# loli/medpy

Measured on AMD Instinct MI355X. Metric: Mvoxels/s graph-cut (build+solve), 512^3 6-conn; fraction of HBM roofline, higher is better.
Workload: dtype f64

## Files before the change

include/medpy_hip.h:

```cpp
#ifndef MEDPY_HIP_H
#define MEDPY_HIP_H

#include <stdint.h>

#ifdef __cplusplus
extern "C" {
#endif

typedef struct mgc_graph* mgc_handle;

typedef enum mgc_status {
    MGC_OK = 0,
    MGC_ERR_INVALID = 1,
    MGC_ERR_NO_DEVICE = 2,
    MGC_ERR_HIP = 3,
    MGC_ERR_OOM = 4,
    MGC_ERR_STATE = 5,
    MGC_ERR_UNSUPPORTED = 6,
    MGC_ERR_NOT_CONVERGED = 7
} mgc_status;

typedef enum mgc_term {
    MGC_TERM_NONE = 0,
    MGC_TERM_DIFFERENCE_LINEAR = 1,
// ... 92 lines not shown
int mgc_get_nweights(mgc_handle h, int axis, double* out);
int mgc_get_tweights(mgc_handle h, double* out);
int mgc_get_nweights_offset(mgc_handle h, const int* offset, double* out);
int mgc_get_edge(mgc_handle h, int64_t i, int64_t j, double* out);

int mgc_maxflow(mgc_handle h, double* flow);

int mgc_labels(mgc_handle h, uint8_t* out);
int mgc_what_segment(mgc_handle h, int64_t i, int* segment);

int mgc_get_node_num(mgc_handle h, int64_t* n);
int mgc_set_param(mgc_handle h, const char* name, int64_t value);
int mgc_get_stats(mgc_handle h, mgc_stats* out);
int mgc_get_profile(mgc_handle h, uint64_t* out16);
enum {
    MGC_LAUNCH_DISCHARGE = 0,
    MGC_LAUNCH_DISCHARGE_W = 1,
    MGC_LAUNCH_RELABEL_TILE = 2,
    MGC_LAUNCH_RELABEL_V = 3,
    MGC_LAUNCH_RELABEL_W = 4,
    MGC_LAUNCH_DISCHARGE26 = 5,
    MGC_LAUNCH_DISCHARGE26_V = 6,
    MGC_LAUNCH_DISCHARGE26_W = 7,
    MGC_NLAUNCH = 8
};
int mgc_get_launch_counts(mgc_handle h, int64_t* out, int n);

enum {
    MGC_OP_ABSORB_ALL = 0,
    MGC_OP_FILL_INF = 1,
    MGC_OP_ZERO_COUNT = 2,
    MGC_OP_RELABEL_ALL = 3,
    MGC_OP_RELABEL_LIST = 4,
    MGC_OP_ACTIVATE = 5,
    MGC_OP_DISCHARGE = 6,
    MGC_OP_SUSPECT_PASS = 7,
    MGC_OP_RESET_SUSPECT = 8
};
int mgc_create_slab(int ndim, const int64_t* global_shape, int connectivity, int device, int rank, int nranks, mgc_handle* out);
int mgc_slab_info(mgc_handle h, int64_t* info8);
int mgc_solver_op(mgc_handle h, int op, int64_t a0, int64_t a1, int64_t a2, int64_t a3);
int mgc_read_counts(mgc_handle h, int32_t* out32);
int mgc_halo_bytes(mgc_handle h, int kind, int64_t* bytes);
int mgc_halo_pack(mgc_handle h, int side, int kind, void* buf, int buf_on_device);
int mgc_halo_unpack(mgc_handle h, int side, int kind, const void* buf, int buf_on_device, uint32_t epoch, int list);
int mgc_finish(mgc_handle h, double* flow_partial);

int mgc_comm_unique_id(uint8_t* id128);
int mgc_comm_init(mgc_handle h, const uint8_t* id128);
int mgc_halo_exchange(mgc_handle h, int kind, uint32_t epoch, int list);

typedef struct mgc_slab_stats {
    int64_t outer;
    int64_t relabel_passes;
    int64_t phases;
    int64_t exchanges;
    int64_t reductions;
    int64_t converged;
    int64_t discharge_tiles;
    int64_t relabel_tiles;
    int64_t deferred_drains;
    int64_t reserved[7];
} mgc_slab_stats;
int mgc_solve_slab(mgc_handle h, mgc_slab_stats* out);

// ... 57 lines not shown
```

medpy_amd/_lib.py:

```python
import ctypes as C
import os

import numpy as np

_HERE = os.path.dirname(os.path.abspath(__file__))
LIB_PATH = os.environ.get("MEDPY_HIP_LIB") or os.path.join(_HERE, "libmedpyhip.so")

OK, ERR_INVALID, ERR_NO_DEVICE, ERR_HIP, ERR_OOM, ERR_STATE, ERR_UNSUPPORTED, ERR_NOT_CONVERGED = range(8)

TERM_IDS = {
    "none": 0,
    "difference_linear": 1, "difference_exponential": 2, "difference_division": 3, "difference_power": 4,
    "maximum_linear": 5, "maximum_exponential": 6, "maximum_division": 7, "maximum_power": 8,
}

DTYPE_IDS = {
    np.dtype(np.uint8): 0, np.dtype(np.int8): 1, np.dtype(np.uint16): 2, np.dtype(np.int16): 3,
    np.dtype(np.uint32): 4, np.dtype(np.int32): 5, np.dtype(np.uint64): 6, np.dtype(np.int64): 7,
    np.dtype(np.float32): 8, np.dtype(np.float64): 9,
}


class Stats(C.Structure):
    _fields_ = [
        ("build_ms", C.c_double), ("solve_ms", C.c_double), ("discharge_ms", C.c_double), ("relabel_ms", C.c_double),
        ("discharge_launches", C.c_int64), ("relabel_launches", C.c_int64), ("discharge_tiles", C.c_int64),
        ("relabel_tiles", C.c_int64), ("global_relabels", C.c_int64), ("phases", C.c_int64), ("ntiles", C.c_int64),
        ("nvox", C.c_int64), ("device_bytes", C.c_int64), ("reserved", C.c_int64 * 3),
        ("discharge_wave_ms", C.c_double), ("discharge_wave_launches", C.c_int64), ("discharge_wave_tiles", C.c_int64),
        ("timing_stride", C.c_int64), ("update_ms", C.c_double), ("delta_ms", C.c_double),
    ]

    def as_dict(self):
        d = {k: getattr(self, k) for k, _ in self._fields_ if k != "reserved"}
        d["readbacks"] = self.reserved[0]
        d["radial_cycles"] = self.reserved[1]
        d["wall_tiles"] = self.reserved[2]
        return d


LAUNCH_KINDS = ("k_discharge", "k_discharge_w", "k_relabel_tile", "k_relabel_v", "k_relabel_w", "k26_discharge", "k26_discharge_v", "k26_discharge_w")


class Validation(C.Structure):
    _fields_ = [("voxels", C.c_int64), ("negative_values", C.c_int64), ("active_excess", C.c_int64),
                ("residual_arcs_across", C.c_int64), ("sink_links_across", C.c_int64), ("pair_violations", C.c_int64),
                ("node_violations", C.c_int64), ("pending_outbox", C.c_int64), ("reserved", C.c_int64 * 4),
                ("max_pair_error", C.c_double), ("max_node_error", C.c_double), ("flow_into_sink", C.c_double),
                ("cut_capacity", C.c_double), ("flow_constant", C.c_double), ("sink_capacity_used", C.c_double),
                ("reserved_d", C.c_double * 2)]

    def as_dict(self):
        return {k: getattr(self, k) for k, _ in self._fields_ if not k.startswith("reserved")}


VIOLATION_KEYS = ("negative_values", "active_excess", "residual_arcs_across", "sink_links_across", "pair_violations",
                  "node_violations", "pending_outbox")


def assert_valid(v, rel=1e-9):
    bad = {k: v[k] for k in VIOLATION_KEYS if v[k]}
    assert not bad, "max-flow invariants violated: %r" % (bad,)
    scale = max(abs(v["flow_into_sink"]), abs(v["cut_capacity"]), 1e-300)
    diff = abs(v["flow_into_sink"] - v["cut_capacity"])
# ... 52 lines not shown
    "mgc_labels_delta": (_INT, [_VP, _I64, _VP, C.POINTER(_I64)]),
    "mgc_add_edges": (_INT, [_VP, _I64, _VP, _VP, _VP, _VP]),
    "mgc_set_tweights_merged": (_INT, [_VP, _VP, _DBL]),
    "mgc_build": (_INT, [_VP]),
    "mgc_get_nweights": (_INT, [_VP, _INT, _VP]),
    "mgc_get_tweights": (_INT, [_VP, _VP]),
    "mgc_get_nweights_offset": (_INT, [_VP, C.POINTER(_INT), _VP]),
    "mgc_get_edge": (_INT, [_VP, _I64, _I64, C.POINTER(_DBL)]),
    "mgc_maxflow": (_INT, [_VP, C.POINTER(_DBL)]),
    "mgc_labels": (_INT, [_VP, _VP]),
    "mgc_what_segment": (_INT, [_VP, _I64, C.POINTER(_INT)]),
    "mgc_get_node_num": (_INT, [_VP, C.POINTER(_I64)]),
    "mgc_set_param": (_INT, [_VP, C.c_char_p, _I64]),
    "mgc_validate": (_INT, [_VP, _VP]),
    "mgc_get_image_range": (_INT, [_VP, _VP]),
    "mgc_set_image_range": (_INT, [_VP, _VP]),
    "mgc_get_stats": (_INT, [_VP, C.POINTER(Stats)]),
    "mgc_get_profile": (_INT, [_VP, _VP]),
    "mgc_get_launch_counts": (_INT, [_VP, _VP, _INT]),
    "mgc_create_slab": (_INT, [_INT, C.POINTER(_I64), _INT, _INT, _INT, _INT, C.POINTER(_VP)]),
    "mgc_slab_info": (_INT, [_VP, C.POINTER(_I64)]),
    "mgc_solver_op": (_INT, [_VP, _INT, _I64, _I64, _I64, _I64]),
    "mgc_read_counts": (_INT, [_VP, _VP]),
    "mgc_halo_bytes": (_INT, [_VP, _INT, C.POINTER(_I64)]),
    "mgc_halo_pack": (_INT, [_VP, _INT, _INT, _VP, _INT]),
    "mgc_halo_unpack": (_INT, [_VP, _INT, _INT, _VP, _INT, C.c_uint32, _INT]),
    "mgc_finish": (_INT, [_VP, C.POINTER(_DBL)]),
    "mgc_comm_unique_id": (_INT, [_VP]),
    "mgc_comm_init": (_INT, [_VP, _VP]),
    "mgc_halo_exchange": (_INT, [_VP, _INT, C.c_uint32, _INT]),
    "mgc_allreduce_counts": (_INT, [_VP, _VP]),
    "mgc_solve_slab": (_INT, [_VP, C.POINTER(SlabStats)]),
    "mgc_solve_slabs": (_INT, [C.POINTER(C.c_void_p), _INT, C.POINTER(Transport), C.POINTER(SlabStats)]),
    "msg_create": (_INT, [_I64, _INT, C.POINTER(_VP)]),
    "msg_destroy": (_INT, [_VP]),
    "msg_last_error": (C.c_char_p, [_VP]),
    "msg_set_param": (_INT, [_VP, C.c_char_p, _I64]),
    "msg_add_edges": (_INT, [_VP, _I64, _VP, _VP, _VP, _VP]),
    "msg_add_lattice_edges": (_INT, [_VP, _INT, _INT, C.POINTER(_I64), _VP, _INT, _DBL, C.POINTER(_DBL)]),
    "msg_add_label_edges": (_INT, [_VP, _INT, _INT, C.POINTER(_I64), _VP, _VP, _INT, _DBL]),
    "msg_region_sums": (_INT, [_INT, _I64, _VP, _VP, _INT, _INT, _I64, _VP, _VP]),
    "msg_set_tweights_merged": (_INT, [_VP, _VP, _DBL]),
    "msg_maxflow": (_INT, [_VP, C.POINTER(_DBL)]),
    "msg_labels": (_INT, [_VP, _VP]),
    "msg_what_segment": (_INT, [_VP, _I64, C.POINTER(_INT)]),
    "msg_get_edge": (_INT, [_VP, _I64, _I64, C.POINTER(_DBL)]),
# ... 76 lines not shown
```

medpy_amd/csrc/mgc_kernels.hip:

```cpp
#include <hip/hip_runtime.h>
#include <rccl/rccl.h>

#include <dlfcn.h>

#include <math.h>
#include <stdarg.h>
#include <stdio.h>
#include <stdlib.h>
#include <string.h>

#include <algorithm>
#include <map>
#include <string>
#include <mutex>
#include <thread>
#include <vector>

#include "../../include/medpy_hip.h"
#include "mgc_tile_ops.inl"
#include "mgc_tile_ops26.inl"
#include "mgc_wave_ops.inl"
#include "mgc_wave_ops26.inl"
#include "mgc_dt_ops.inl"
#include "mgc_brick_ops.inl"
// ... 798 lines not shown

__global__ __launch_bounds__(MGC_TV) void k_activate_list(MgcLattice L, int list, int cnt, uint32_t phase)
{
    __shared__ MgcTileShared S;
    GpuBlock x(S);
    MgcListView view;
    const int n = mgc_list_view(L, cnt, view);
    for (int i = blockIdx.x; i < n; i += gridDim.x) {
        x.new_tile();
        mgc_activate_tile(x, L, mgc_list_at(L, list, view, i), phase);
        __syncthreads();
    }
}

template <int AXIS, bool BWD, int SEED, int FINAL>
__global__ __launch_bounds__(256) void k_dt_scan(MgcLattice L, const void* in, void* out, int c_min, int32_t* hout, const uint16_t* carry_in, uint16_t* carry_out, int carry_plane)
{
    __shared__ MgcWaveShared S;
    GpuWave w(S);
    const int n = mgc_dt_lines<AXIS>(L);
    for (int line = (int)blockIdx.x * 4 + (int)(threadIdx.x >> 6); line < n; line += (int)gridDim.x * 4) {
        w.new_tile();
        mgc_dt_scan_line<AXIS, BWD, SEED, FINAL>(w, L, __builtin_amdgcn_readfirstlane(line), in, out, c_min, hout, carry_in, carry_out, carry_plane);
    }
}

__global__ __launch_bounds__(256) void k_shadow_sync(MgcLattice L)
{
    __shared__ MgcWaveShared S;
    GpuWave w(S);
    const int T = L.gy * L.gx;
    for (int i = (int)blockIdx.x * 4 + (int)(threadIdx.x >> 6); i < 2 * T; i += (int)gridDim.x * 4) {
        w.new_tile();
        mgc_shadow_sync_tile(w, L, i / T, __builtin_amdgcn_readfirstlane(i % T), L.height);
    }
}

__global__ __launch_bounds__(256) void k_dt_finish(MgcLattice L)
{
    __shared__ MgcWaveShared S;
    GpuWave w(S);
    if (blockIdx.x == 0 && threadIdx.x == 0) atomicAdd(&L.count[9], L.ntiles);
    for (int tile = (int)blockIdx.x * 4 + (int)(threadIdx.x >> 6); tile < L.ntiles; tile += (int)gridDim.x * 4) {
        w.new_tile();
        mgc_dt_finish_tile(w, L, __builtin_amdgcn_readfirstlane(tile));
    }
// ... 1647 lines not shown
            else hipLaunchKernelGGL(k_absorb_list, dim3(grid(h->L.ntiles)), dim3(MGC_TV), 0, h->stream, h->L, 6, fslot(0), fnext(0));
            filter_done(0, true);
            check(hipGetLastError());
        }
    }
    void relabel_all(uint32_t epoch, int next)
    {
        flush_zero();
        h->brick_mode = false;
        const int id = time_begin(1);
        if constexpr (FULL) hipLaunchKernelGGL(k26_relabel_all, dim3(grid(h->L.ntiles)), dim3(MGC_TV), 0, h->stream, h->L, epoch, next);
        else if (!(h->use_filters & 1)) { hipLaunchKernelGGL(k_relabel_all, dim3(grid(h->L.ntiles)), dim3(MGC_TV), 0, h->stream, h->L, epoch, next); h->launches[MGC_LAUNCH_RELABEL_TILE]++; }
        else {
            flush_zero();
            hipLaunchKernelGGL(k_filter, dim3(filter_grid()), dim3(256), 0, h->stream, h->L, 3, 6, fslot(0));
            if (h->wave_kernels & 8) { hipLaunchKernelGGL(k_relabel_v, dim3(grid(h->L.ntiles)), dim3(MGC_TV / MGC_RELABEL_V), 0, h->stream, h->L, 6, fslot(0), epoch, next, fnext(0), 1); filter_done(0, true); h->launches[MGC_LAUNCH_RELABEL_V]++; }
            else if (h->wave_kernels & 2) { hipLaunchKernelGGL(k_relabel_w, dim3(h->wave_grid_rel), dim3(MGCW_LANES), 0, h->stream, h->L, 6, fslot(0), epoch, next, -1, 1, h->tk_rel); h->tk_rel ^= 1; filter_done(0, false); h->launches[MGC_LAUNCH_RELABEL_W]++; }
            else { hipLaunchKernelGGL(k_relabel_first_list, dim3(grid(h->L.ntiles)), dim3(MGC_TV), 0, h->stream, h->L, 6, fslot(0), epoch, next); filter_done(0, false); h->launches[MGC_LAUNCH_RELABEL_TILE]++; }
        }
        check(hipGetLastError());
        time_end(id);
        relabel_launches++;
    }
    bool first_relabel_dt()
    {
        if (FULL || !h->use_dt || !h->all_residual || h->labels_valid || h->nranks > 1) return false;
        if (!h->d_dt16) {
            if (mgc_dmalloc((void**)&h->d_dt16, (size_t)h->L.ntiles * MGC_TV * sizeof(uint16_t)) != hipSuccess) { (void)hipGetLastError(); return false; }
            h->device_bytes += (int64_t)h->L.ntiles * MGC_TV * (int64_t)sizeof(uint16_t);
        }
        flush_zero();
        h->labels_valid = true;
        const int id = time_begin(2);
        const MgcLattice& L = h->L;
        void* const T = h->d_dt16;
        const dim3 blk(256);
        auto g = [&](int lines) { return dim3(grid((lines + 3) / 4)); };
        hipLaunchKernelGGL((k_dt_scan<0, false, 1, 0>), g(L.gz * L.gy), blk, 0, h->stream, L, (const void*)L.rmask, T, 0, (int32_t*)nullptr, (const uint16_t*)nullptr, (uint16_t*)nullptr, -1);
        hipLaunchKernelGGL((k_dt_scan<0, true, 0, 0>), g(L.gz * L.gy), blk, 0, h->stream, L, (const void*)T, T, 0, (int32_t*)nullptr, (const uint16_t*)nullptr, (uint16_t*)nullptr, -1);
        hipLaunchKernelGGL((k_dt_scan<1, false, 0, 0>), g(L.gz * L.gx), blk, 0, h->stream, L, (const void*)T, T, 0, (int32_t*)nullptr, (const uint16_t*)nullptr, (uint16_t*)nullptr, -1);
        hipLaunchKernelGGL((k_dt_scan<1, true, 0, 0>), g(L.gz * L.gx), blk, 0, h->stream, L, (const void*)T, T, 0, (int32_t*)nullptr, (const uint16_t*)nullptr, (uint16_t*)nullptr, -1);
        hipLaunchKernelGGL((k_dt_scan<2, false, 0, 0>), g(L.gy * L.gx), blk, 0, h->stream, L, (const void*)T, T, 0, (int32_t*)nullptr, (const uint16_t*)nullptr, (uint16_t*)nullptr, -1);
        hipLaunchKernelGGL((k_dt_scan<2, true, 0, 1>), g(L.gy * L.gx), blk, 0, h->stream, L, (const void*)T, (void*)L.height, 0, (int32_t*)nullptr, (const uint16_t*)nullptr, (uint16_t*)nullptr, -1);
        hipLaunchKernelGGL(k_dt_finish, g(L.ntiles), blk, 0, h->stream, L);
        check(hipGetLastError());
        time_end(id);
        relabel_launches += 7;
        return true;
    }
    void set_radial(bool on) { h->radial_on = on; if (on) h->radial_cycle_no++; }
    bool radial_begin(int c_min)
    {
        if (FULL) return false;
        const size_t nv = (size_t)h->L.ntiles * MGC_TV;
        if (!h->d_ds16) {
            if (mgc_dmalloc((void**)&h->d_ds16, nv * sizeof(uint16_t)) != hipSuccess) { (void)hipGetLastError(); return false; }
            h->device_bytes += (int64_t)(nv * sizeof(uint16_t));
        }
        if (!h->d_hexact) {
            if (mgc_dmalloc((void**)&h->d_hexact, nv * sizeof(int32_t)) != hipSuccess) { (void)hipGetLastError(); return false; }
            h->device_bytes += (int64_t)(nv * sizeof(int32_t));
        }
        flush_zero();
        const int id = time_begin(2);
        const MgcLattice& L = h->L;
        void* const T = h->d_ds16;
        const dim3 blk(256);
        auto g = [&](int lines) { return dim3(grid((lines + 3) / 4)); };
        check(hipMemsetAsync(L.count + mgc_cnt_radial_c(L), 0x3f, sizeof(int32_t), h->stream));
        hipLaunchKernelGGL(k_dt_cmin, g(L.ntiles), blk, 0, h->stream, L);
        hipLaunchKernelGGL((k_dt_scan<0, false, 2, 0>), g(L.gz * L.gy), blk, 0, h->stream, L, (const void*)L.excess, T, 0, (int32_t*)nullptr, (const uint16_t*)nullptr, (uint16_t*)nullptr, -1);
        hipLaunchKernelGGL((k_dt_scan<0, true, 0, 0>), g(L.gz * L.gy), blk, 0, h->stream, L, (const void*)T, T, 0, (int32_t*)nullptr, (const uint16_t*)nullptr, (uint16_t*)nullptr, -1);
        hipLaunchKernelGGL((k_dt_scan<1, false, 0, 0>), g(L.gz * L.gx), blk, 0, h->stream, L, (const void*)T, T, 0, (int32_t*)nullptr, (const uint16_t*)nullptr, (uint16_t*)nullptr, -1);
        hipLaunchKernelGGL((k_dt_scan<1, true, 0, 0>), g(L.gz * L.gx), blk, 0, h->stream, L, (const void*)T, T, 0, (int32_t*)nullptr, (const uint16_t*)nullptr, (uint16_t*)nullptr, -1);
        hipLaunchKernelGGL((k_dt_scan<2, false, 0, 0>), g(L.gy * L.gx), blk, 0, h->stream, L, (const void*)T, T, 0, (int32_t*)nullptr, (const uint16_t*)nullptr, (uint16_t*)nullptr, -1);
        hipLaunchKernelGGL((k_dt_scan<2, true, 0, 2>), g(L.gy * L.gx), blk, 0, h->stream, L, (const void*)T, T, c_min, h->d_hexact, (const uint16_t*)nullptr, (uint16_t*)nullptr, -1);
        std::swap(h->L.height, h->d_hexact);
        check(hipGetLastError());
        time_end(id);
        relabel_launches += 8;
        return true;
    }
    void radial_save_exact()
    {
        flush_zero();
        check(hipMemcpyAsync(h->d_hexact, h->L.height, (size_t)h->L.ntiles * MGC_TV * sizeof(int32_t), hipMemcpyDeviceToDevice, h->stream));
    }
    void radial_restore_exact()
    {
        flush_zero();
        std::swap(h->L.height, h->d_hexact);
    }
    void radial_lower(int c_min)
    {
        flush_zero();
        const int id = time_begin(2);
        hipLaunchKernelGGL(k_dt_lower, dim3(grid((h->L.ntiles + 3) / 4)), dim3(256), 0, h->stream, h->L, (const uint16_t*)h->d_ds16, c_min);
        check(hipGetLastError());
        time_end(id);
        relabel_launches++;
    }
    void source_open()
    {
// ... 104 lines not shown
    uint16_t* carry_buf(int dir) { return h->d_carry[dir]; }
    uint16_t* carry_recv_buf(int dir) { return h->d_carry_in[dir]; }
    bool ensure(void** p, size_t bytes)
    {
        if (*p) return true;
        if (mgc_dmalloc(p, bytes) != hipSuccess) { (void)hipGetLastError(); *p = nullptr; return false; }
        h->device_bytes += (int64_t)bytes;
        return true;
    }
    bool dt_applicable()
    {
        if (FULL || !h->use_dt || !h->all_residual || h->labels_valid) return false;
        bool ok = ensure((void**)&h->d_dt16, (size_t)h->L.ntiles * MGC_TV * sizeof(uint16_t));
        for (int k = 0; k < 2 && ok; ++k) ok = ensure((void**)&h->d_carry[k], (size_t)carry_bytes()) && ensure((void**)&h->d_carry_in[k], (size_t)carry_bytes());
        return ok;
    }
    dim3 dt_grid(int lines) const { return dim3(grid((lines + 3) / 4)); }
    int dt_span = -1;
    void dt_scans_xy(int seed)
    {
        flush_zero();
        h->labels_valid = true;
        dt_span = time_begin(2);
        const MgcLattice& L = h->L;
        void* const T = h->dt_cur = seed == 1 ? h->d_dt16 : h->d_ds16;
        const dim3 blk(256);
        if (seed == 1) hipLaunchKernelGGL((k_dt_scan<0, false, 1, 0>), dt_grid(L.gz * L.gy), blk, 0, h->stream, L, (const void*)L.rmask, T, 0, (int32_t*)nullptr, (const uint16_t*)nullptr, (uint16_t*)nullptr, -1);
        else hipLaunchKernelGGL((k_dt_scan<0, false, 2, 0>), dt_grid(L.gz * L.gy), blk, 0, h->stream, L, (const void*)L.excess, T, 0, (int32_t*)nullptr, (const uint16_t*)nullptr, (uint16_t*)nullptr, -1);
        hipLaunchKernelGGL((k_dt_scan<0, true, 0, 0>), dt_grid(L.gz * L.gy), blk, 0, h->stream, L, (const void*)T, T, 0, (int32_t*)nullptr, (const uint16_t*)nullptr, (uint16_t*)nullptr, -1);
        hipLaunchKernelGGL((k_dt_scan<1, false, 0, 0>), dt_grid(L.gz * L.gx), blk, 0, h->stream, L, (const void*)T, T, 0, (int32_t*)nullptr, (const uint16_t*)nullptr, (uint16_t*)nullptr, -1);
        hipLaunchKernelGGL((k_dt_scan<1, true, 0, 0>), dt_grid(L.gz * L.gx), blk, 0, h->stream, L, (const void*)T, T, 0, (int32_t*)nullptr, (const uint16_t*)nullptr, (uint16_t*)nullptr, -1);
        check(hipGetLastError());
        relabel_launches += 4;
    }
    void dt_scan_z(bool bwd, int final_kind, int c_min, const uint16_t* cin, bool want_out)
    {
        const MgcLattice& L = h->L;
        void* const T = h->dt_cur;
        const dim3 blk(256), g = dt_grid(L.gy * L.gx);
        uint16_t* const cout = want_out ? h->d_carry[bwd ? 1 : 0] : nullptr;
        const int plane = want_out ? carry_plane(bwd ? 1 : 0) : -1;
        if (!bwd) hipLaunchKernelGGL((k_dt_scan<2, false, 0, 0>), g, blk, 0, h->stream, L, (const void*)T, T, 0, (int32_t*)nullptr, cin, cout, plane);
        else if (final_kind == 1) hipLaunchKernelGGL((k_dt_scan<2, true, 0, 1>), g, blk, 0, h->stream, L, (const void*)T, (void*)L.height, 0, (int32_t*)nullptr, cin, cout, plane);
        else if (final_kind == 2) hipLaunchKernelGGL((k_dt_scan<2, true, 0, 2>), g, blk, 0, h->stream, L, (const void*)T, T, c_min, h->d_hexact, cin, cout, plane);
        else hipLaunchKernelGGL((k_dt_scan<2, true, 0, 0>), g, blk, 0, h->stream, L, (const void*)T, T, 0, (int32_t*)nullptr, cin, cout, plane);
        check(hipGetLastError());
        relabel_launches++;
        if (bwd) { time_end(dt_span); dt_span = -1; }
    }
    void dt_finish()
    {
        hipLaunchKernelGGL(k_dt_finish, dt_grid(h->L.ntiles), dim3(256), 0, h->stream, h->L);
        check(hipGetLastError());
        relabel_launches++;
    }
    void shadow_sync()
    {
        if (FULL || (!has_lower() && !has_upper())) return;
        hipLaunchKernelGGL(k_shadow_sync, dt_grid(2 * h->L.gy * h->L.gx), dim3(256), 0, h->stream, h->L);
        check(hipGetLastError());
    }
    bool radial_prepare()
    {
        if (FULL) return false;
        const size_t nv = (size_t)h->L.ntiles * MGC_TV;
        return ensure((void**)&h->d_ds16, nv * sizeof(uint16_t)) && ensure((void**)&h->d_hexact, nv * sizeof(int32_t));
    }
    void radial_cmin()
    {
        flush_zero();
// ... 127 lines not shown
        while (h->op_ev.size() < need) {
            hipEvent_t e;
            if (hipEventCreate(&e) != hipSuccess) break;
            h->op_ev.push_back(e);
        }
        if (h->op_ev.size() >= need) {
            ev_a = (int)(2 * h->op_spans.size());
            (void)hipEventRecord(h->op_ev[ev_a], h->stream);
        }
    }
    switch (op) {
    case MGC_OP_ABSORB_ALL: dev.absorb_all(); break;
    case MGC_OP_FILL_INF: dev.fill_heights_inf(); break;
    case MGC_OP_ZERO_COUNT:
        if (a0 < 0 || a0 >= MGC_NCOUNT) { h->timing = timing; return mgc_fail(h, MGC_ERR_INVALID, "counter index"); }
        dev.zero_count((int)a0);
        break;
    case MGC_OP_RELABEL_ALL: dev.relabel_all((uint32_t)a0, (int)a1); break;
    case MGC_OP_RELABEL_LIST: dev.relabel_list((int)a0, (uint32_t)a1, (int)a2); break;
    case MGC_OP_ACTIVATE: dev.activate_all((uint32_t)a0); break;
    case MGC_OP_DISCHARGE: dev.discharge((int)a0, (uint32_t)a1, (int)a2, (int)a3); break;
    case MGC_OP_SUSPECT_PASS: dev.suspect_pass(); break;
    case MGC_OP_RESET_SUSPECT: dev.reset_suspect((uint32_t)a0, (int)a1); break;
    default: h->timing = timing; return mgc_fail(h, MGC_ERR_INVALID, "unknown solver op %d", op);
    }
    if (ev_a >= 0) {
        (void)hipEventRecord(h->op_ev[ev_a + 1], h->stream);
        h->op_spans.push_back({ev_a, ev_a + 1, span_kind});
    }
    h->timing = timing;
    h->solved = false;
    if (dev.first_error != hipSuccess) return mgc_fail(h, MGC_ERR_HIP, "solver op %d: %s", op, hipGetErrorString(dev.first_error));
    return MGC_OK;
}


static void mgc_sum_partials(mgc_handle h, int64_t n, double* out)
{
    if (n > 8192 && h->d_part2) {
        const int64_t len = (n + 255) / 256;
        hipLaunchKernelGGL(k_sum_chunks, dim3(256), dim3(256), 0, h->stream, (const double*)h->d_part, n, len, h->d_part2);
        hipLaunchKernelGGL(k_sum_partials, dim3(1), dim3(MGC_TV), 0, h->stream, (const double*)h->d_part2, (int64_t)256, out);
    } else {
        hipLaunchKernelGGL(k_sum_partials, dim3(1), dim3(MGC_TV), 0, h->stream, (const double*)h->d_part, n, out);
    }
}
// ... 1473 lines not shown
    else if (!strcmp(name, "check_rounds") && value > 0) h->params.check_rounds = (int)value;
    else if (!strcmp(name, "stop_below") && value >= 0) h->params.stop_below = (int)value;
    else if (!strcmp(name, "incremental_relabel")) h->params.incremental_relabel = value != 0;
    else if (!strcmp(name, "trace")) h->params.trace = value != 0;
    else if (!strcmp(name, "adaptive_rounds") && value >= 0) h->params.adaptive_rounds = (int)value;
    else if (!strcmp(name, "radial") && value >= 0 && value <= 2) h->params.radial = (int)value;
    else if (!strcmp(name, "radial_min_walls") && value >= 0) h->radial_min_walls = (int)value;
    else if (!strcmp(name, "radial_budget_x16") && value >= 1) h->params.radial_budget_x16 = (int)value;
    else if (!strcmp(name, "radial_min_c") && value >= 1) h->params.radial_min_c = (int)value;
    else if (!strcmp(name, "radial_rounds0") && value >= 0) h->params.radial_rounds0 = (int)value;
    else if (!strcmp(name, "use_filters") && value >= 0 && value <= 7) h->use_filters = (int)value;
    else if (!strcmp(name, "wave_kernels") && value >= 0 && value <= 63) { h->wave_kernels = (int)value; h->wave_set = true; }
    else if (!strcmp(name, "wave_min_tiles") && value >= 0) h->wave_min_tiles = (int)value;
    else if (!strcmp(name, "sweeps_sparse26") && value >= 0) { h->sweeps_sparse26 = (int)value; h->sparse26_set = true; }
    else if (!strcmp(name, "wave_grid_dis") && value > 0) h->wave_grid_dis = (int)value;
    else if (!strcmp(name, "wave_grid26") && value > 0) h->wave_grid26 = (int)value;
    else if (!strcmp(name, "prepush")) h->prepush = value != 0;
    else if ((!strcmp(name, "exchange_passes") || !strcmp(name, "relabel_exchange_every")) && value > 0) h->params.exchange_passes = (int)value;
    else if (!strcmp(name, "exchange_rounds") && value > 0) h->params.exchange_rounds = (int)value;
    else if (!strcmp(name, "w26_passes") && value > 0) h->w26_passes = (int)value;
    else if (!strcmp(name, "w26_raises") && value > 0) h->w26_raises = (int)value;
    else if (!strcmp(name, "w26_flags") && value >= 0) h->w26_flags = (int)value;
    else if (!strcmp(name, "wave_grid_rel") && value > 0) h->wave_grid_rel = (int)value;
    else if (!strcmp(name, "first_relabel_dt")) h->use_dt = value != 0;
    else if (!strcmp(name, "relabel_bricks")) h->use_bricks = value != 0;
    else if (!strcmp(name, "exact_sink_tiles") && value >= 0 && value <= 2) h->exact_sink_tiles = (int)value;
    else if (!strcmp(name, "sink_sweeps") && value > 0) h->sink_sweeps = (int)value;
    else if (!strcmp(name, "halo_max_records") && value >= 1) {
        const int64_t T = (int64_t)h->L.gy * h->L.gx;
        h->L.halo_max_rec = (int)(value < T ? value : T);
    }
    else if (!strcmp(name, "wave_stagger") && value >= 0) h->wave_stagger = (int)value;
    else if (!strcmp(name, "repeat_steps") && value >= 0 && value <= 7) h->repeat_steps = (int)value;
    else if (!strcmp(name, "repeat_min_tiles") && value >= 0) h->repeat_min_tiles = (int)value;
    else if (!strcmp(name, "repeat_flood_min_tiles") && value >= 0) h->repeat_flood_min_tiles = (int)value;
    else if (!strcmp(name, "list_shards") && (value == 1 || value == MGC_NSHARD)) {
        mgc_flush_zero(h);
        MGC_HIP(h, hipMemsetAsync(h->L.count, 0, MGC_NCOUNT * (1 + MGC_NSHARD) * sizeof(int32_t), h->stream));
        h->L.nshard = (int)value;
        h->filt[0] = h->filt[1] = 0;
        h->solved = false;
    }
    else if (!strcmp(name, "activate_exact_max") && value >= 0) h->activate_exact_max = (int)value;
    else if (!strcmp(name, "kernel_timing")) h->timing = value != 0;
    else if (!strcmp(name, "timing_stride") && value > 0) h->timing_stride = (int)value;
    else if (!strcmp(name, "profile_sections")) {
        if (value && !h->L.prof) {
// ... 3 lines not shown
        if (!value && h->L.prof) { (void)mgc_dfree(h->L.prof); h->L.prof = nullptr; }
    }
    else return mgc_fail(h, MGC_ERR_INVALID, "unknown or invalid parameter %s=%lld", name, (long long)value);
    return MGC_OK;
}

int mgc_get_profile(mgc_handle h, uint64_t* out16)
{
    if (!h || !out16) return MGC_ERR_INVALID;
    memset(out16, 0, 16 * sizeof(uint64_t));
    if (!h->L.prof) return MGC_OK;
    MGC_HIP(h, hipSetDevice(h->device));
    MGC_HIP(h, hipMemcpy(out16, h->L.prof, 16 * sizeof(uint64_t), hipMemcpyDeviceToHost));
    return MGC_OK;
}

int mgc_get_launch_counts(mgc_handle h, int64_t* out, int n)
{
    if (!h || !out || n < 0) return MGC_ERR_INVALID;
    for (int k = 0; k < n && k < MGC_NLAUNCH; ++k) out[k] = h->launches[k];
    return MGC_OK;
}

int mgc_get_stats(mgc_handle h, mgc_stats* out)
{
    if (!h || !out) return MGC_ERR_INVALID;
    h->stats.ntiles = h->L.ntiles;
    h->stats.nvox = h->nvox;
    h->stats.device_bytes = h->device_bytes;
    *out = h->stats;
    return MGC_OK;
}

}
```

medpy_amd/graphcut/graph.py:

```python
import ctypes as C
import enum

import numpy

from .. import _lib


class termtype(enum.IntEnum):
    SOURCE = 0
    SINK = 1


def _holds_whole_numbers(image, block=1 << 20):
    flat = image.reshape(-1) if image.flags.c_contiguous else image.ravel()
    for start in range(0, flat.size, block):
        part = flat[start:start + block]
        if not numpy.array_equal(part, numpy.floor(part)):
            return False
    return True


def image_table_facts(term, image):
    import math
    if not (term.endswith("exponential") or term.endswith("power")):
# ... 276 lines not shown
        shp = list(self._shape)
        shp[axis] -= 1
        out = numpy.empty(shp, dtype=numpy.float64)
        if out.size:
            self._call("mgc_get_nweights", int(axis), _lib.ptr(out))
        return out

    def tweights(self):
        out = numpy.empty(self._shape, dtype=numpy.float64)
        self._call("mgc_get_tweights", _lib.ptr(out))
        return out

    def profile(self):
        out = numpy.zeros(16, dtype=numpy.uint64)
        self._call("mgc_get_profile", _lib.ptr(out))
        names = ("load", "labels", "sweep", "store", "votes", "faceflags", "s6", "s7")
        return {n: {"cycles": int(out[i]), "count": int(out[i + 8])} for i, n in enumerate(names)}

    def stats(self):
        st = _lib.Stats()
        self._call("mgc_get_stats", C.byref(st))
        return st.as_dict()

    def launch_counts(self):
        out = numpy.zeros(len(_lib.LAUNCH_KINDS), dtype=numpy.int64)
        self._call("mgc_get_launch_counts", _lib.ptr(out), int(out.size))
        return dict(zip(_lib.LAUNCH_KINDS, out.tolist()))


class SparseGraph(object):

    termtype = termtype
    _captype = "double"

    @staticmethod
    def _cast(v):
        return float(v)

    @classmethod
    def _out(cls, v):
        return cls._cast(v)

    def __init__(self, nodes, edges=0, device=0):
        lib = _lib.load()
        if _lib.device_count() < 1:
            raise _lib.MedpyHipError(_lib.ERR_NO_DEVICE, "no HIP device visible; medpy_amd has no CPU fallback")
# ... 680 lines not shown
```

medpy_amd/slab.py:

```python
import numpy as np

(OP_ABSORB_ALL, OP_FILL_INF, OP_ZERO_COUNT, OP_RELABEL_ALL, OP_RELABEL_LIST, OP_ACTIVATE, OP_DISCHARGE, OP_SUSPECT_PASS,
 OP_RESET_SUSPECT) = range(9)


class LoopbackExchange(object):

    def __init__(self, slabs):
        self.slabs = list(slabs)

    def allreduce_sum(self, values):
        return np.sum(np.asarray(values, dtype=np.float64), axis=0)

    def allreduce_max(self, values):
        return np.max(np.asarray(values, dtype=np.float64), axis=0)


class StoreExchange(object):

    def __init__(self, slab, store):
        self.store, self.slabs = store, [slab]
        self.rank, self.world = store.rank, store.world

    def xchg(self, lo, hi):
# ... 267 lines not shown

    def allreduce_counts(self):
        out = np.zeros(32, dtype=np.int64)
        self._call("mgc_allreduce_counts", self._lib.ptr(out))
        return out

    def finish_device(self):
        f = self._C.c_double(0.0)
        self._call("mgc_finish", self._C.byref(f))
        return f.value

    def finish(self):
        f = self._C.c_double(self.finish_device())
        out = np.empty(int(np.prod(self.local_shape)), dtype=np.uint8)
        self._call("mgc_labels", self._lib.ptr(out))
        lab = out.reshape(self.local_shape)[self.own0 - self.plane0:self.own1 - self.plane0].astype(np.bool_)
        return lab, f.value

    def stats(self):
        st = self._lib.Stats()
        self._call("mgc_get_stats", self._C.byref(st))
        return st.as_dict()

    def validate(self):
        v = self._lib.Validation()
        self._call("mgc_validate", self._C.byref(v))
        return v.as_dict()


def validate_slabs(slabs, ex):
    from . import _lib
    parts = [s.validate() for s in slabs]
    keys = [k for k in parts[0] if k not in ("max_pair_error", "max_node_error")]
    sums = np.asarray(ex.allreduce_sum([[float(p[k]) for k in keys] for p in parts]), dtype=np.float64).reshape(-1)
    mx = np.asarray(ex.allreduce_max([[p["max_pair_error"], p["max_node_error"]] for p in parts]), dtype=np.float64).reshape(-1)
    out = {k: (float(v) if k in ("flow_into_sink", "cut_capacity", "flow_constant", "sink_capacity_used") else int(round(v))) for k, v in zip(keys, sums)}
    out["max_pair_error"], out["max_node_error"] = float(mx[0]), float(mx[1])
    return out


def graphcut_voxel_slabs(image, fg, bg, term="difference_exponential", sigma=None, spacing=False, nslabs=2, device=0,
                         connectivity=6, regional=None, **schedule):
    image, fg, bg = np.asarray(image), np.asarray(fg), np.asarray(bg)
    slabs = [HipSlab(image.shape, r, nslabs, device=device, connectivity=connectivity) for r in range(nslabs)]
    for s in slabs:
        sl = slice(s.plane0, s.plane1)
# ... 22 lines not shown
```

Measured before the change: 7379.

## Fuse forward and backward distance-transform scans into one per-axis kernel

Adds a k_dt_axis kernel in which each wavefront holds an 8-tile run of a line in registers, does the forward and backward min-plus scans locally, and merges the ends of the runs across waves through shared memory. The first-relabel and radial-relabel distance transforms then launch one kernel per axis instead of two. This halves the launches and the read/write passes over the 16-bit distance buffer. The old two-scan path stays as a fallback for long axes or when use_dt is 2, and the change also adds debug entry points (a first-relabel op, height readback, launch counters).

```diff
diff --git a/include/medpy_hip.h b/include/medpy_hip.h
--- a/include/medpy_hip.h
+++ b/include/medpy_hip.h
@@ -138,7 +138,9 @@
     MGC_LAUNCH_DISCHARGE26 = 5,
     MGC_LAUNCH_DISCHARGE26_V = 6,
     MGC_LAUNCH_DISCHARGE26_W = 7,
-    MGC_NLAUNCH = 8
+    MGC_LAUNCH_DT_AXIS = 8,
+    MGC_LAUNCH_DT_SCAN = 9,
+    MGC_NLAUNCH = 10
 };
 int mgc_get_launch_counts(mgc_handle h, int64_t* out, int n);
 
@@ -151,12 +153,14 @@
     MGC_OP_ACTIVATE = 5,
     MGC_OP_DISCHARGE = 6,
     MGC_OP_SUSPECT_PASS = 7,
-    MGC_OP_RESET_SUSPECT = 8
+    MGC_OP_RESET_SUSPECT = 8,
+    MGC_OP_FIRST_RELABEL = 9
 };
 int mgc_create_slab(int ndim, const int64_t* global_shape, int connectivity, int device, int rank, int nranks, mgc_handle* out);
 int mgc_slab_info(mgc_handle h, int64_t* info8);
 int mgc_solver_op(mgc_handle h, int op, int64_t a0, int64_t a1, int64_t a2, int64_t a3);
 int mgc_read_counts(mgc_handle h, int32_t* out32);
+int mgc_get_heights(mgc_handle h, int which, int32_t* out);
 int mgc_halo_bytes(mgc_handle h, int kind, int64_t* bytes);
 int mgc_halo_pack(mgc_handle h, int side, int kind, void* buf, int buf_on_device);
 int mgc_halo_unpack(mgc_handle h, int side, int kind, const void* buf, int buf_on_device, uint32_t epoch, int list);
diff --git a/medpy_amd/_lib.py b/medpy_amd/_lib.py
--- a/medpy_amd/_lib.py
+++ b/medpy_amd/_lib.py
@@ -39,7 +39,11 @@
         return d
 
 
-LAUNCH_KINDS = ("k_discharge", "k_discharge_w", "k_relabel_tile", "k_relabel_v", "k_relabel_w", "k26_discharge", "k26_discharge_v", "k26_discharge_w")
+OP_FIRST_RELABEL = 9
+HINF = 0x3f3f3f3f
+
+LAUNCH_KINDS = ("k_discharge", "k_discharge_w", "k_relabel_tile", "k_relabel_v", "k_relabel_w", "k26_discharge", "k26_discharge_v", "k26_discharge_w",
+                "k_dt_axis", "k_dt_scan")
 
 
 class Validation(C.Structure):
@@ -138,6 +142,7 @@
     "mgc_slab_info": (_INT, [_VP, C.POINTER(_I64)]),
     "mgc_solver_op": (_INT, [_VP, _INT, _I64, _I64, _I64, _I64]),
     "mgc_read_counts": (_INT, [_VP, _VP]),
+    "mgc_get_heights": (_INT, [_VP, _INT, _VP]),
     "mgc_halo_bytes": (_INT, [_VP, _INT, C.POINTER(_I64)]),
     "mgc_halo_pack": (_INT, [_VP, _INT, _INT, _VP, _INT]),
     "mgc_halo_unpack": (_INT, [_VP, _INT, _INT, _VP, _INT, C.c_uint32, _INT]),
diff --git a/medpy_amd/csrc/mgc_kernels.hip b/medpy_amd/csrc/mgc_kernels.hip
--- a/medpy_amd/csrc/mgc_kernels.hip
+++ b/medpy_amd/csrc/mgc_kernels.hip
@@ -844,6 +844,118 @@
     for (int line = (int)blockIdx.x * 4 + (int)(threadIdx.x >> 6); line < n; line += (int)gridDim.x * 4) {
         w.new_tile();
         mgc_dt_scan_line<AXIS, BWD, SEED, FINAL>(w, L, __builtin_amdgcn_readfirstlane(line), in, out, c_min, hout, carry_in, carry_out, carry_plane);
+    }
+}
+
+#define MGC_DT_RUN 8
+#define MGC_DT_MAXW 16
+#define MGC_DT_BIG (1 << 20)
+template <int AXIS, int SEED, int FINAL>
+__global__ __launch_bounds__(64 * MGC_DT_MAXW) void k_dt_axis(MgcLattice L, const void* in, void* out, int c_min, int32_t* hout, int W, int LPB)
+{
+    __shared__ int s_end[2][MGC_DT_MAXW][2][64];
+    const int l = (int)(threadIdx.x & 63u);
+    const int wv = __builtin_amdgcn_readfirstlane((int)(threadIdx.x >> 6));
+    const int sub = wv / W, j = wv - sub * W;
+    const int n = mgc_dt_lines<AXIS>(L);
+    const int na = AXIS == 0 ? L.gx : (AXIS == 1 ? L.gy : L.gz);
+    const int64_t len = AXIS == 0 ? L.dx : (AXIS == 1 ? L.dy : L.dz);
+    const int t0 = j * MGC_DT_RUN;
+    const int nt = na - t0 < MGC_DT_RUN ? na - t0 : MGC_DT_RUN;
+    const int ngroups = (n + LPB - 1) / LPB;
+    int C = MGC_HINF;
+    if (FINAL == 2) { C = L.count[mgc_cnt_radial_c(L)]; if (C < c_min) C = MGC_HINF; }
+    int half = 0;
+    for (int grp = (int)blockIdx.x; grp < ngroups; grp += (int)gridDim.x, half ^= 1) {
+        const int line = grp * LPB + sub;
+        const bool have = line < n;
+        int v[MGC_DT_RUN][8];
+        int64_t room = 0;
+        if (have) {
+            int64_t cu, cv, du, dv;
+            if (AXIS == 0) { cu = (int64_t)(line / L.gy) * 8 + (l >> 3); cv = (int64_t)(line % L.gy) * 8 + (l & 7); du = L.dz; dv = L.dy; }
+            else if (AXIS == 1) { cu = (int64_t)(line / L.gx) * 8 + (l >> 3); cv = (int64_t)(line % L.gx) * 8 + (l & 7); du = L.dz; dv = L.dx; }
+            else { cu = (int64_t)(line / L.gx) * 8 + (l >> 3); cv = (int64_t)(line % L.gx) * 8 + (l & 7); du = L.dy; dv = L.dx; }
+            room = cu < du && cv < dv ? len - (int64_t)t0 * 8 : 0;
+#pragma unroll
+            for (int g = 0; g < MGC_DT_RUN; ++g) {
+                const int tile = g < nt ? mgc_dt_tile<AXIS>(L, line, t0 + g) : -1;
+                if (tile >= 0 && (SEED != 2 || mgc_source_tile(L, tile))) {
+                    const int64_t base = (int64_t)tile * MGC_TV;
+#pragma unroll
+                    for (int i = 0; i < 8; ++i) {
+                        const int loc = mgc_dt_loc<AXIS>(l, i);
+                        if (SEED == 1) v[g][i] = (((const uint8_t*)in)[base + loc] & MGC_MASK_SINK) ? 1 : MGC_DT_INF;
+                        else if (SEED == 2) v[g][i] = ((const double*)in)[base + loc] > 0.0 ? 1 : MGC_DT_INF;
+                        else v[g][i] = ((const uint16_t*)in)[base + loc];
+                    }
+                } else {
+#pragma unroll
+                    for (int i = 0; i < 8; ++i) v[g][i] = MGC_DT_INF;
+                }
+            }
+            int c = MGC_DT_BIG;
+#pragma unroll
+            for (int g = 0; g < MGC_DT_RUN; ++g)
+#pragma unroll
+                for (int i = 0; i < 8; ++i) {
+                    if (g * 8 + i >= room) v[g][i] = MGC_DT_INF;
+                    c = v[g][i] < c + 1 ? v[g][i] : c + 1;
+                    v[g][i] = c;
+                }
+            c = MGC_DT_BIG;
+#pragma unroll
+            for (int g = MGC_DT_RUN - 1; g >= 0; --g)
+#pragma unroll
+                for (int i = 7; i >= 0; --i) {
+                    c = v[g][i] < c + 1 ? v[g][i] : c + 1;
+                    v[g][i] = c;
+                }
+            s_end[half][wv][0][l] = v[MGC_DT_RUN - 1][7];
+            s_end[half][wv][1][l] = v[0][0];
+        }
+        __syncthreads();
+        if (!have) continue;
+        int ef = MGC_DT_BIG, eb = MGC_DT_BIG;
+        for (int k = 0; k < j; ++k) { const int e = s_end[half][sub * W + k][0][l]; ef = e < ef + 64 ? e : ef + 64; }
+        for (int k = W - 1; k > j; --k) { const int e = s_end[half][sub * W + k][1][l]; eb = e < eb + 64 ? e : eb + 64; }
+        int hx[2][8];
+        if (FINAL == 2) {
+            const int64_t base = (int64_t)mgc_dt_tile<AXIS>(L, line, t0) * MGC_TV;
+#pragma unroll
+            for (int i = 0; i < 8; ++i) hx[0][i] = L.height[base + mgc_dt_loc<AXIS>(l, i)];
+        }
+#pragma unroll
+        for (int g = 0; g < MGC_DT_RUN; ++g) {
+            if (g >= nt) break;
+            const int64_t base = (int64_t)mgc_dt_tile<AXIS>(L, line, t0 + g) * MGC_TV;
+            if (FINAL == 2 && g + 1 < nt) {
+                const int64_t nbase = (int64_t)mgc_dt_tile<AXIS>(L, line, t0 + g + 1) * MGC_TV;
+#pragma unroll
+                for (int i = 0; i < 8; ++i) hx[(g + 1) & 1][i] = L.height[nbase + mgc_dt_loc<AXIS>(l, i)];
+            }
+#pragma unroll
+            for (int i = 0; i < 8; ++i) {
+                const int p = g * 8 + i, loc = mgc_dt_loc<AXIS>(l, i);
+                int val = v[g][i];
+                val = val < ef + 1 + p ? val : ef + 1 + p;
+                val = val < eb + 64 - p ? val : eb + 64 - p;
+                if (val > MGC_DT_INF || p >= room) val = MGC_DT_INF;
+                if (FINAL == 1) ((int32_t*)out)[base + loc] = val < MGC_DT_INF ? val : MGC_HINF;
+                else ((uint16_t*)out)[base + loc] = (uint16_t)val;
+                if (FINAL == 2 && (hout || (C < MGC_HINF && val < MGC_DT_INF))) {
+                    const int hv = hx[g & 1][i];
+                    int nv = hv;
+                    if (C < MGC_HINF && val < MGC_DT_INF) {
+                        int gl = C - mgc_radial_steps(L, val - 1);
+                        gl = gl < 1 ? 1 : gl;
+                        if (hv < MGC_HINF && gl < hv) nv = gl;
+                    }
+                    if (hout) hout[base + loc] = nv;
+                    else if (nv != hv) L.height[base + loc] = nv;
+                }
+            }
+        }
     }
 }
 
@@ -2537,6 +2649,27 @@
         time_end(id);
         relabel_launches++;
     }
+    template <int AXIS, int SEED, int FINAL>
+    void dt_axis(const void* in, uint16_t* T, int c_min)
+    {
+        const MgcLattice& L = h->L;
+        const int lines = mgc_dt_lines<AXIS>(L), na = AXIS == 0 ? L.gx : (AXIS == 1 ? L.gy : L.gz);
+        void* const out = FINAL == 1 ? (void*)L.height : (void*)T;
+        int32_t* const hout = FINAL == 2 ? h->d_hexact : nullptr;
+        const int W = (na + MGC_DT_RUN - 1) / MGC_DT_RUN;
+        if (h->use_dt != 2 && W <= MGC_DT_MAXW) {
+            const int LPB = W >= 4 ? 1 : 4 / W;
+            hipLaunchKernelGGL((k_dt_axis<AXIS, SEED, FINAL>), dim3(grid((lines + LPB - 1) / LPB)), dim3(64 * W * LPB), 0, h->stream, L, in, out, c_min, hout, W, LPB);
+            h->launches[MGC_LAUNCH_DT_AXIS]++;
+            relabel_launches++;
+            return;
+        }
+        const dim3 g(grid((lines + 3) / 4)), blk(256);
+        hipLaunchKernelGGL((k_dt_scan<AXIS, false, SEED, 0>), g, blk, 0, h->stream, L, in, (void*)T, 0, (int32_t*)nullptr, (const uint16_t*)nullptr, (uint16_t*)nullptr, -1);
+        hipLaunchKernelGGL((k_dt_scan<AXIS, true, 0, FINAL>), g, blk, 0, h->stream, L, (const void*)T, out, c_min, hout, (const uint16_t*)nullptr, (uint16_t*)nullptr, -1);
+        h->launches[MGC_LAUNCH_DT_SCAN] += 2;
+        relabel_launches += 2;
+    }
     bool first_relabel_dt()
     {
         if (FULL || !h->use_dt || !h->all_residual || h->labels_valid || h->nranks > 1) return false;
@@ -2548,19 +2681,16 @@
         h->labels_valid = true;
         const int id = time_begin(2);
         const MgcLattice& L = h->L;
-        void* const T = h->d_dt16;
+        uint16_t* const T = h->d_dt16;
         const dim3 blk(256);
         auto g = [&](int lines) { return dim3(grid((lines + 3) / 4)); };
-        hipLaunchKernelGGL((k_dt_scan<0, false, 1, 0>), g(L.gz * L.gy), blk, 0, h->stream, L, (const void*)L.rmask, T, 0, (int32_t*)nullptr, (const uint16_t*)nullptr, (uint16_t*)nullptr, -1);
-        hipLaunchKernelGGL((k_dt_scan<0, true, 0, 0>), g(L.gz * L.gy), blk, 0, h->stream, L, (const void*)T, T, 0, (int32_t*)nullptr, (const uint16_t*)nullptr, (uint16_t*)nullptr, -1);
-        hipLaunchKernelGGL((k_dt_scan<1, false, 0, 0>), g(L.gz * L.gx), blk, 0, h->stream, L, (const void*)T, T, 0, (int32_t*)nullptr, (const uint16_t*)nullptr, (uint16_t*)nullptr, -1);
-        hipLaunchKernelGGL((k_dt_scan<1, true, 0, 0>), g(L.gz * L.gx), blk, 0, h->stream, L, (const void*)T, T, 0, (int32_t*)nullptr, (const uint16_t*)nullptr, (uint16_t*)nullptr, -1);
-        hipLaunchKernelGGL((k_dt_scan<2, false, 0, 0>), g(L.gy * L.gx), blk, 0, h->stream, L, (const void*)T, T, 0, (int32_t*)nullptr, (const uint16_t*)nullptr, (uint16_t*)nullptr, -1);
-        hipLaunchKernelGGL((k_dt_scan<2, true, 0, 1>), g(L.gy * L.gx), blk, 0, h->stream, L, (const void*)T, (void*)L.height, 0, (int32_t*)nullptr, (const uint16_t*)nullptr, (uint16_t*)nullptr, -1);
+        dt_axis<0, 1, 0>((const void*)L.rmask, T, 0);
+        dt_axis<1, 0, 0>((const void*)T, T, 0);
+        dt_axis<2, 0, 1>((const void*)T, T, 0);
         hipLaunchKernelGGL(k_dt_finish, g(L.ntiles), blk, 0, h->stream, L);
         check(hipGetLastError());
         time_end(id);
-        relabel_launches += 7;
+        relabel_launches++;
         return true;
     }
     void set_radial(bool on) { h->radial_on = on; if (on) h->radial_cycle_no++; }
@@ -2579,21 +2709,18 @@
         flush_zero();
         const int id = time_begin(2);
         const MgcLattice& L = h->L;
-        void* const T = h->d_ds16;
+        uint16_t* const T = h->d_ds16;
         const dim3 blk(256);
         auto g = [&](int lines) { return dim3(grid((lines + 3) / 4)); };
         check(hipMemsetAsync(L.count + mgc_cnt_radial_c(L), 0x3f, sizeof(int32_t), h->stream));
         hipLaunchKernelGGL(k_dt_cmin, g(L.ntiles), blk, 0, h->stream, L);
-        hipLaunchKernelGGL((k_dt_scan<0, false, 2, 0>), g(L.gz * L.gy), blk, 0, h->stream, L, (const void*)L.excess, T, 0, (int32_t*)nullptr, (const uint16_t*)nullptr, (uint16_t*)nullptr, -1);
-        hipLaunchKernelGGL((k_dt_scan<0, true, 0, 0>), g(L.gz * L.gy), blk, 0, h->stream, L, (const void*)T, T, 0, (int32_t*)nullptr, (const uint16_t*)nullptr, (uint16_t*)nullptr, -1);
-        hipLaunchKernelGGL((k_dt_scan<1, false, 0, 0>), g(L.gz * L.gx), blk, 0, h->stream, L, (const void*)T, T, 0, (int32_t*)nullptr, (const uint16_t*)nullptr, (uint16_t*)nullptr, -1);
-        hipLaunchKernelGGL((k_dt_scan<1, true, 0, 0>), g(L.gz * L.gx), blk, 0, h->stream, L, (const void*)T, T, 0, (int32_t*)nullptr, (const uint16_t*)nullptr, (uint16_t*)nullptr, -1);
-        hipLaunchKernelGGL((k_dt_scan<2, false, 0, 0>), g(L.gy * L.gx), blk, 0, h->stream, L, (const void*)T, T, 0, (int32_t*)nullptr, (const uint16_t*)nullptr, (uint16_t*)nullptr, -1);
-        hipLaunchKernelGGL((k_dt_scan<2, true, 0, 2>), g(L.gy * L.gx), blk, 0, h->stream, L, (const void*)T, T, c_min, h->d_hexact, (const uint16_t*)nullptr, (uint16_t*)nullptr, -1);
+        dt_axis<0, 2, 0>((const void*)L.excess, T, 0);
+        dt_axis<1, 0, 0>((const void*)T, T, 0);
+        dt_axis<2, 0, 2>((const void*)T, T, c_min);
         std::swap(h->L.height, h->d_hexact);
         check(hipGetLastError());
         time_end(id);
-        relabel_launches += 8;
+        relabel_launches++;
         return true;
     }
     void radial_save_exact()
@@ -2744,16 +2871,11 @@
         flush_zero();
         h->labels_valid = true;
         dt_span = time_begin(2);
-        const MgcLattice& L = h->L;
-        void* const T = h->dt_cur = seed == 1 ? h->d_dt16 : h->d_ds16;
-        const dim3 blk(256);
-        if (seed == 1) hipLaunchKernelGGL((k_dt_scan<0, false, 1, 0>), dt_grid(L.gz * L.gy), blk, 0, h->stream, L, (const void*)L.rmask, T, 0, (int32_t*)nullptr, (const uint16_t*)nullptr, (uint16_t*)nullptr, -1);
-        else hipLaunchKernelGGL((k_dt_scan<0, false, 2, 0>), dt_grid(L.gz * L.gy), blk, 0, h->stream, L, (const void*)L.excess, T, 0, (int32_t*)nullptr, (const uint16_t*)nullptr, (uint16_t*)nullptr, -1);
-        hipLaunchKernelGGL((k_dt_scan<0, true, 0, 0>), dt_grid(L.gz * L.gy), blk, 0, h->stream, L, (const void*)T, T, 0, (int32_t*)nullptr, (const uint16_t*)nullptr, (uint16_t*)nullptr, -1);
-        hipLaunchKernelGGL((k_dt_scan<1, false, 0, 0>), dt_grid(L.gz * L.gx), blk, 0, h->stream, L, (const void*)T, T, 0, (int32_t*)nullptr, (const uint16_t*)nullptr, (uint16_t*)nullptr, -1);
-        hipLaunchKernelGGL((k_dt_scan<1, true, 0, 0>), dt_grid(L.gz * L.gx), blk, 0, h->stream, L, (const void*)T, T, 0, (int32_t*)nullptr, (const uint16_t*)nullptr, (uint16_t*)nullptr, -1);
+        uint16_t* const T = h->dt_cur = seed == 1 ? h->d_dt16 : h->d_ds16;
+        if (seed == 1) dt_axis<0, 1, 0>((const void*)h->L.rmask, T, 0);
+        else dt_axis<0, 2, 0>((const void*)h->L.excess, T, 0);
+        dt_axis<1, 0, 0>((const void*)T, T, 0);
         check(hipGetLastError());
-        relabel_launches += 4;
     }
     void dt_scan_z(bool bwd, int final_kind, int c_min, const uint16_t* cin, bool want_out)
     {
@@ -2768,6 +2890,7 @@
         else hipLaunchKernelGGL((k_dt_scan<2, true, 0, 0>), g, blk, 0, h->stream, L, (const void*)T, T, 0, (int32_t*)nullptr, cin, cout, plane);
         check(hipGetLastError());
         relabel_launches++;
+        h->launches[MGC_LAUNCH_DT_SCAN]++;
         if (bwd) { time_end(dt_span); dt_span = -1; }
     }
     void dt_finish()
@@ -2941,6 +3064,11 @@
     case MGC_OP_DISCHARGE: dev.discharge((int)a0, (uint32_t)a1, (int)a2, (int)a3); break;
     case MGC_OP_SUSPECT_PASS: dev.suspect_pass(); break;
     case MGC_OP_RESET_SUSPECT: dev.reset_suspect((uint32_t)a0, (int)a1); break;
+    case MGC_OP_FIRST_RELABEL:
+        for (int64_t& n : h->launches) n = 0;
+        if (h->nranks > 1 || !dev.first_relabel_dt()) { h->timing = timing; return mgc_fail(h, MGC_ERR_STATE, "the distance transform does not apply to this graph (a slab, first_relabel_dt = 0, an n-link that is not residual, or labels this build already has)"); }
+        if (a0 && !dev.radial_begin((int)a1)) { h->timing = timing; return mgc_fail(h, MGC_ERR_STATE, "no radial labels on this graph"); }
+        break;
     default: h->timing = timing; return mgc_fail(h, MGC_ERR_INVALID, "unknown solver op %d", op);
     }
     if (ev_a >= 0) {
@@ -4460,7 +4588,7 @@
     else if (!strcmp(name, "w26_raises") && value > 0) h->w26_raises = (int)value;
     else if (!strcmp(name, "w26_flags") && value >= 0) h->w26_flags = (int)value;
     else if (!strcmp(name, "wave_grid_rel") && value > 0) h->wave_grid_rel = (int)value;
-    else if (!strcmp(name, "first_relabel_dt")) h->use_dt = value != 0;
+    else if (!strcmp(name, "first_relabel_dt") && value >= 0 && value <= 2) h->use_dt = (int)value;
     else if (!strcmp(name, "relabel_bricks")) h->use_bricks = value != 0;
     else if (!strcmp(name, "exact_sink_tiles") && value >= 0 && value <= 2) h->exact_sink_tiles = (int)value;
     else if (!strcmp(name, "sink_sweeps") && value > 0) h->sink_sweeps = (int)value;
@@ -4510,6 +4638,27 @@
     return MGC_OK;
 }
 
+int mgc_get_heights(mgc_handle h, int which, int32_t* out)
+{
+    if (!h || !out || which < 0 || which > 1) return MGC_ERR_INVALID;
+    if (!h->built || h->nranks > 1) return mgc_fail(h, MGC_ERR_STATE, "mgc_get_heights: a built single handle");
+    const MgcLattice& L = h->L;
+    const int32_t* const src = which ? h->d_hexact : L.height;
+    if (!src) return mgc_fail(h, MGC_ERR_STATE, "mgc_get_heights: no label array is kept aside");
+    MGC_HIP(h, hipSetDevice(h->device));
+    mgc_flush_zero(h);
+    std::vector<int32_t> tiled((size_t)L.ntiles * MGC_TV);
+    MGC_HIP(h, hipMemcpyAsync(tiled.data(), src, tiled.size() * sizeof(int32_t), hipMemcpyDeviceToHost, h->stream));
+    MGC_HIP(h, hipStreamSynchronize(h->stream));
+    for (int64_t z = 0; z < L.dz; ++z)
+        for (int64_t y = 0; y < L.dy; ++y)
+            for (int64_t x = 0; x < L.dx; ++x) {
+                const int64_t tile = ((z >> 3) * L.gy + (y >> 3)) * L.gx + (x >> 3);
+                out[(z * L.dy + y) * L.dx + x] = tiled[(size_t)(tile * MGC_TV + (z & 7) * 64 + (y & 7) * 8 + (x & 7))];
+            }
+    return MGC_OK;
+}
+
 int mgc_get_stats(mgc_handle h, mgc_stats* out)
 {
     if (!h || !out) return MGC_ERR_INVALID;
diff --git a/medpy_amd/graphcut/graph.py b/medpy_amd/graphcut/graph.py
--- a/medpy_amd/graphcut/graph.py
+++ b/medpy_amd/graphcut/graph.py
@@ -322,6 +322,14 @@
         self._call("mgc_get_stats", C.byref(st))
         return st.as_dict()
 
+    def first_relabel(self, radial=False, c_min=8):
+        self._call("mgc_solver_op", _lib.OP_FIRST_RELABEL, 1 if radial else 0, int(c_min), 0, 0)
+
+    def heights(self, aside=False):
+        out = numpy.empty(self._shape, dtype=numpy.int32)
+        self._call("mgc_get_heights", 1 if aside else 0, _lib.ptr(out))
+        return out
+
     def launch_counts(self):
         out = numpy.zeros(len(_lib.LAUNCH_KINDS), dtype=numpy.int64)
         self._call("mgc_get_launch_counts", _lib.ptr(out), int(out.size))
diff --git a/medpy_amd/slab.py b/medpy_amd/slab.py
--- a/medpy_amd/slab.py
+++ b/medpy_amd/slab.py
@@ -313,6 +313,11 @@
         self._call("mgc_get_stats", self._C.byref(st))
         return st.as_dict()
 
+    def launch_counts(self):
+        out = np.zeros(len(self._lib.LAUNCH_KINDS), dtype=np.int64)
+        self._call("mgc_get_launch_counts", self._lib.ptr(out), int(out.size))
+        return dict(zip(self._lib.LAUNCH_KINDS, out.tolist()))
+
     def validate(self):
         v = self._lib.Validation()
         self._call("mgc_validate", self._C.byref(v))
```

New measurement: 7640, median of 6. 1.04x the previous value.
